# DeepMETv2/DeepMETv2

Hardware: AMD Instinct MI355X
Metric: events/sec (4.5k PF cands, k=16) (higher is better)
Workload: dtype f32

## Files before the change

### deepmetv2_amd/build.py

```python
from __future__ import annotations

import concurrent.futures as cf
import os
import shutil
import subprocess
import sys

PKG_DIR = os.path.dirname(os.path.abspath(__file__))
CSRC = os.path.join(PKG_DIR, "csrc")
OBJ_DIR = os.path.join(CSRC, "_obj")
LIB_PATH = os.path.join(PKG_DIR, "libdmet_hip.so")
SOURCES = ["knn.hip", "radius.hip", "edgeconv.hip", "edgemlp.hip", "misc.hip", "dense.hip", "encoder.hip", "norm.hip", "edgeconv_bwd.hip",
           "head.hip", "finalize.hip", "pool.hip",
           "edgemlp_f32.hip", "edgemlp_bf16.hip", "edgeconv_sum.hip", "gravnet.hip", "attention.hip", "fps.hip", "interpolate.hip",
           "pointnet.hip", "gat.hip", "segment.hip", "multi_aggr.hip", "weighted_sum.hip", "event_norm.hip", "select.hip"]
HEADERS = [os.path.join(CSRC, h) for h in ("common.h", "bn_affine.h", "knn_common.h", "knn_filter.h", "knn_key64.h", "nls_body.h",
                                           "edgemlp_fused.h", "row_softmax.h")] + \
          [os.path.join(PKG_DIR, "..", "include", "dmet.h")]
ARCH = "gfx950"
CXXFLAGS = ["-O3", "-std=c++17", "-fPIC", f"--offload-arch={ARCH}", "-ffp-contract=off", "-Wall",
            "-Wno-unused-function", "-DNDEBUG"]


def _hipcc() -> str:
    exe = shutil.which("hipcc") or "/opt/rocm/bin/hipcc"
    if not os.path.exists(exe):
        raise RuntimeError("hipcc not found: cannot build libdmet_hip.so")
    return exe


def _stale(target: str, deps) -> bool:
    if not os.path.exists(target):
        return True
    t = os.path.getmtime(target)
    return any(os.path.getmtime(d) > t for d in deps if os.path.exists(d))


def _compile(src: str, force: bool) -> str:
    obj = os.path.join(OBJ_DIR, os.path.splitext(src)[0] + ".o")
    path = os.path.join(CSRC, src)
    if force or _stale(obj, [path] + HEADERS):
        cmd = [_hipcc()] + CXXFLAGS + ["-c", path, "-o", obj]
        subprocess.check_call(cmd)
    return obj


def build_hip(force: bool = False, verbose: bool = False) -> str:
    os.makedirs(OBJ_DIR, exist_ok=True)
    with cf.ThreadPoolExecutor(max_workers=min(4, len(SOURCES))) as ex:
        objs = list(ex.map(lambda s: _compile(s, force), SOURCES))
    if force or _stale(LIB_PATH, objs):
        cmd = [_hipcc(), "-shared", "-fPIC", f"--offload-arch={ARCH}", "-o", LIB_PATH] + objs
        if verbose:
            print(" ".join(cmd))
        subprocess.check_call(cmd)
    return LIB_PATH


if __name__ == "__main__":
    print(build_hip(force="--force" in sys.argv, verbose=True))
```

### deepmetv2_amd/csrc/knn.hip

```cpp
#include <stdlib.h>

#include "common.h"
#include "knn_common.h"
#include "knn_key64.h"
#include "nls_body.h"

namespace dmet {
namespace {

constexpr int kTileC = 32;
constexpr int kQMax = 8;
constexpr int kMaxSplit = 8;
constexpr int kWavesPerGroup = 4;

#define DMET_PKSUB_LO " op_sel:[0,0] op_sel_hi:[0,1] neg_lo:[0,1] neg_hi:[0,1]\n\t"
#define DMET_PKSUB_HI " op_sel:[1,0] op_sel_hi:[1,1] neg_lo:[0,1] neg_hi:[0,1]\n\t"
__device__ __forceinline__ void pk_dist_step4(f2 &accA, f2 &accB, f2 vxy, f2 vzw, f2 wxy, f2 wzw, f2 q0, f2 q1, f2 q2,
                                              f2 q3)
{
    f2 t0, t1, t2, t3;
    asm("v_pk_add_f32 %[t0], %[vxy], %[q0]" DMET_PKSUB_LO
        "v_pk_add_f32 %[t1], %[wxy], %[q0]" DMET_PKSUB_LO
        "v_pk_add_f32 %[t2], %[vxy], %[q1]" DMET_PKSUB_HI
        "v_pk_add_f32 %[t3], %[wxy], %[q1]" DMET_PKSUB_HI
        "v_pk_fma_f32 %[a], %[t0], %[t0], %[a]\n\t"
        "v_pk_fma_f32 %[b], %[t1], %[t1], %[b]\n\t"
        "v_pk_add_f32 %[t0], %[vzw], %[q2]" DMET_PKSUB_LO
        "v_pk_add_f32 %[t1], %[wzw], %[q2]" DMET_PKSUB_LO
        "v_pk_fma_f32 %[a], %[t2], %[t2], %[a]\n\t"
        "v_pk_fma_f32 %[b], %[t3], %[t3], %[b]\n\t"
        "v_pk_add_f32 %[t2], %[vzw], %[q3]" DMET_PKSUB_HI
        "v_pk_add_f32 %[t3], %[wzw], %[q3]" DMET_PKSUB_HI
        "v_pk_fma_f32 %[a], %[t0], %[t0], %[a]\n\t"
        "v_pk_fma_f32 %[b], %[t1], %[t1], %[b]\n\t"
        "v_pk_fma_f32 %[a], %[t2], %[t2], %[a]\n\t"
        "v_pk_fma_f32 %[b], %[t3], %[t3], %[b]"
        : [a] "+v"(accA), [b] "+v"(accB), [t0] "=&v"(t0), [t1] "=&v"(t1), [t2] "=&v"(t2), [t3] "=&v"(t3)
        : [vxy] "v"(vxy), [vzw] "v"(vzw), [wxy] "v"(wxy), [wzw] "v"(wzw), [q0] "v"(q0), [q1] "v"(q1), [q2] "v"(q2),
          [q3] "v"(q3));
}

template <bool HI>
__device__ __forceinline__ void pk_sub2(f2 &tA, f2 &tB, f2 v, f2 w, f2 q)
{
    if (HI)
        asm("v_pk_add_f32 %[ta], %[v], %[q]" DMET_PKSUB_HI "v_pk_add_f32 %[tb], %[w], %[q]" DMET_PKSUB_HI
            : [ta] "=&v"(tA), [tb] "=&v"(tB) : [v] "v"(v), [w] "v"(w), [q] "v"(q));
    else
        asm("v_pk_add_f32 %[ta], %[v], %[q]" DMET_PKSUB_LO "v_pk_add_f32 %[tb], %[w], %[q]" DMET_PKSUB_LO
            : [ta] "=&v"(tA), [tb] "=&v"(tB) : [v] "v"(v), [w] "v"(w), [q] "v"(q));
}

__device__ __forceinline__ void pk_fma2(f2 &accA, f2 &accB, f2 tA, f2 tB)
{
    asm("v_pk_fma_f32 %[a], %[ta], %[ta], %[a]\n\t"
        "v_pk_fma_f32 %[b], %[tb], %[tb], %[b]"
        : [a] "+v"(accA), [b] "+v"(accB) : [ta] "v"(tA), [tb] "v"(tB));
}

__device__ __forceinline__ float wrap1(float d, float L)
{
    float a, t;
    asm("v_sub_f32 %[t], %[L], |%[d]|\n\t"
        "v_min_f32 %[a], |%[d]|, %[t]"
        : [a] "=v"(a), [t] "=&v"(t) : [d] "v"(d), [L] "s"(L));
    return a;
}

template <bool HI>
__device__ __forceinline__ void pk_dist_step1_per(f2 &accA, f2 &accB, f2 v, f2 w, f2 q, float L, bool wrap)
{
    f2 tA, tB;
    pk_sub2<HI>(tA, tB, v, w, q);
    if (wrap) {
        tA = f2{wrap1(tA.x, L), wrap1(tA.y, L)};
        tB = f2{wrap1(tB.x, L), wrap1(tB.y, L)};
    }
    pk_fma2(accA, accB, tA, tB);
}

template <int DP, int TQ>
struct KnnShared {
    float4 tile[(kTileC + 1) * DP / 4];
    uint2 queue[TQ][kQMax][kWave];
};

template <int KP>
__device__ __attribute__((noinline)) float drain_queue(const uint2 (*queue)[kWave], int lane, int cnt, bool fresh,
                                                       bool valid, float *__restrict__ ld,
                                                       int32_t *__restrict__ lj)
{
    float d[KP];
    int32_t j[KP];
    if (fresh || !valid) {
#pragma unroll
        for (int p = 0; p < KP; ++p) { d[p] = kKnnSentinel; j[p] = -1; }
    } else {
#pragma unroll
        for (int p = 0; p < KP; p += 4) {
            const float4 v = *reinterpret_cast<const float4 *>(ld + p);
            const int4 w = *reinterpret_cast<const int4 *>(lj + p);
            d[p] = v.x; d[p + 1] = v.y; d[p + 2] = v.z; d[p + 3] = v.w;
            j[p] = w.x; j[p + 1] = w.y; j[p + 2] = w.z; j[p + 3] = w.w;
        }
    }
    int maxcnt = cnt;
#pragma unroll
    for (int off = 32; off > 0; off >>= 1) maxcnt = max(maxcnt, __shfl_xor(maxcnt, off, 64));
    for (int s = 0; s < maxcnt; ++s) {
        if (s < cnt) {
            const uint2 e = queue[s][lane];
            const float nd = __uint_as_float(e.x);
            const int32_t nj = (int32_t)e.y;
            if (nd < d[KP - 1]) {
#pragma unroll
                for (int p = KP - 1; p >= 1; --p) {
                    const bool mq = d[p - 1] > nd;
                    const bool mp = d[p] > nd;
                    const float dn = mq ? d[p - 1] : (mp ? nd : d[p]);
                    const int32_t jn = mq ? j[p - 1] : (mp ? nj : j[p]);
                    d[p] = dn;
                    j[p] = jn;
                }
                if (d[0] > nd) { d[0] = nd; j[0] = nj; }
            }
        }
    }
    if (valid) {
#pragma unroll
        for (int p = 0; p < KP; p += 4) {
            *reinterpret_cast<float4 *>(ld + p) = make_float4(d[p], d[p + 1], d[p + 2], d[p + 3]);
            *reinterpret_cast<int4 *>(lj + p) = make_int4(j[p], j[p + 1], j[p + 2], j[p + 3]);
        }
    }
    return d[KP - 1];
}

#ifdef DMET_KNN_STAMP
__device__ unsigned long long g_knn_stamps[1 << 16][4];
#endif

#ifndef DMET_F2_MIN_NODES
#define DMET_F2_MIN_NODES 800
#endif
constexpr int kF2MinNodes = DMET_F2_MIN_NODES;
constexpr int kFilterMaxSplit = 2;
#ifndef DMET_F2_SPLIT_MIN_NODES
#define DMET_F2_SPLIT_MIN_NODES 2560
#endif
constexpr int kF2SplitMinNodes = DMET_F2_SPLIT_MIN_NODES;
constexpr int kF2MaxNodes = 65536;

struct KnnPlan {
    int total_tiles;
    int n_full;
    int split;
    int form1_events;
};

struct KnnArgs {
    const float *x;
    const int64_t *ptr;
    int B;
    int64_t N;
    int D, k;
    int32_t *nbr;
    float *dist;
    uint16_t *nbr16;
    float *wsd;
    int32_t *wsj;
    const KnnPlan *plan;
    const int32_t *order;
    const int32_t *tile_ptr;
    float *psd;
    int32_t *psj;
    const int32_t *flags;
    int flag_min;
    const int32_t *any;
    const int32_t *qlist;
    const int32_t *pos_of;
    int requery_groups;
    int requery_tile_queries;
};

__device__ __forceinline__ uint16_t local_id16(int32_t j, int ev_lo)
{
    return (uint16_t)(j >= 0 ? (unsigned)(j - ev_lo) : 0xFFFFu);
}

constexpr int kMaxSortedEvents = 4096;

struct KnnPlanOut {
    int tile_queries, simds, max_split;
    int32_t *order, *pos_of, *tile_ptr;
    KnnPlan *plan;
};

__device__ __forceinline__ int xcd_dealt_position(int rank, int B)
{
    if (B < 4 * kNumXcd) return rank;
    const int c = rank % (2 * kNumXcd), g = rank / (2 * kNumXcd);
    const int bin = c < kNumXcd ? c : 2 * kNumXcd - 1 - c;
    const int idx = 2 * g + (c >= kNumXcd ? 1 : 0);
    const int rem = B % (2 * kNumXcd), full = B / (2 * kNumXcd);
    int start = 0;
    for (int b = 0; b < bin; ++b)
        start += 2 * full + (b < min(rem, kNumXcd) ? 1 : 0) + ((rem > kNumXcd && b > 2 * kNumXcd - 1 - rem) ? 1 : 0);
    return start + idx;
}

template <bool XY = false>
__device__ __forceinline__ void knn_plan_body(const int64_t *__restrict__ ptr, int B, const KnnPlanOut &o,
                                              const int64_t *__restrict__ cptr = nullptr)
{
    const int tile_queries = o.tile_queries, simds = o.simds, max_split = o.max_split;
    int32_t *__restrict__ order = o.order, *__restrict__ pos_of = o.pos_of, *__restrict__ tile_ptr = o.tile_ptr;
    KnnPlan *__restrict__ plan = o.plan;
    __shared__ int part[256];
    const int tid = threadIdx.x;
    if (B <= kMaxSortedEvents) {
        for (int b = tid; b < B; b += 256) {
            const int64_t nb = ptr[b + 1] - ptr[b];
            int rank = 0;
            if constexpr (XY) {
                const int64_t xb = nb > 0 ? cptr[b + 1] - cptr[b] : -1;
                for (int c = 0; c < B; ++c) {
                    const int64_t nc = ptr[c + 1] - ptr[c];
                    const int64_t xc = nc > 0 ? cptr[c + 1] - cptr[c] : -1;
                    rank += (xc > xb || (xc == xb && (nc > nb || (nc == nb && c < b)))) ? 1 : 0;
                }
            } else {
                for (int c = 0; c < B; ++c) {
                    const int64_t nc = ptr[c + 1] - ptr[c];
                    rank += (nc > nb || (nc == nb && c < b)) ? 1 : 0;
                }
            }
            const int p = xcd_dealt_position(rank, B);
            order[p] = b;
            pos_of[b] = p;
        }
    } else {
        for (int b = tid; b < B; b += 256) { order[b] = b; pos_of[b] = b; }
    }
    __syncthreads();
    const int chunk = (B + 255) / 256;
    const int lo = min(B, tid * chunk), hi = min(B, lo + chunk);
    int sum = 0, nf1 = 0;
    for (int p = lo; p < hi; ++p) {
        const int b = order[p];
        const int64_t nb = ptr[b + 1] - ptr[b];
        sum += (int)((nb + tile_queries - 1) / tile_queries);
        nf1 += (nb > 0 && !(nb >= kF2MinNodes && nb <= kF2MaxNodes)) ? 1 : 0;
    }
    __shared__ unsigned long long xy_cand;
    __shared__ int xy_events;
    if constexpr (XY) {
        if (tid == 0) { xy_cand = 0ull; xy_events = 0; }
        __syncthreads();
        unsigned long long cand = 0ull;
        int evs = 0;
        for (int p = lo; p < hi; ++p) {
            const int b = order[p];
            if (ptr[b + 1] > ptr[b]) { cand += (unsigned long long)(cptr[b + 1] - cptr[b]); ++evs; }
        }
        if (evs) { atomicAdd(&xy_cand, cand); atomicAdd(&xy_events, evs); }
    }
    __shared__ int wave_tot[4], wave_f1[4];
    const int lane = tid & 63, wv = tid >> 6;
    int incl = sum, f1 = nf1;
#pragma unroll
    for (int off = 1; off < 64; off <<= 1) {
        const int t = __shfl_up(incl, off, 64);
        if (lane >= off) incl += t;
    }
#pragma unroll
    for (int off = 32; off > 0; off >>= 1) f1 += __shfl_xor(f1, off, 64);
    if (lane == 63) wave_tot[wv] = incl;
    if (lane == 0) wave_f1[wv] = f1;
    __syncthreads();
    int base = 0;
    for (int w = 0; w < wv; ++w) base += wave_tot[w];
    part[tid] = base + incl - sum;
    if (tid == 0) {
        const int form1_events = wave_f1[0] + wave_f1[1] + wave_f1[2] + wave_f1[3];
        const int tiles = wave_tot[0] + wave_tot[1] + wave_tot[2] + wave_tot[3];
        int n_full = tiles, split = 1;
        const int full = (tiles / simds) * simds;
        const int rem = tiles - full;
        bool cut = rem > 0;
        if constexpr (XY) cut = cut && xy_events > 0 && xy_cand >= 512ull * (unsigned long long)xy_events;
        else cut = cut && B > 0 && (ptr[B] - ptr[0]) >= (int64_t)512 * B;
        if (cut) {
            int f = simds / rem;
            if (f > max_split) f = max_split;
            if (f >= 2) { n_full = full; split = f; }
        }
        plan->total_tiles = tiles; plan->n_full = n_full; plan->split = split; plan->form1_events = form1_events;
        tile_ptr[B] = tiles;
    }
    __syncthreads();
    int run = part[tid];
    for (int p = lo; p < hi; ++p) {
        const int b = order[p];
        tile_ptr[p] = run;
        run += (int)((ptr[b + 1] - ptr[b] + tile_queries - 1) / tile_queries);
    }
    if (o.max_split == kFilterMaxSplit) {
// ... 968 lines not shown
```

### deepmetv2_amd/csrc/knn_filter.h

```cpp
constexpr int kFQ = 64;

typedef float f32x16 __attribute__((ext_vector_type(16)));
typedef short bf16x8 __attribute__((ext_vector_type(8)));
typedef _Float16 f16x8 __attribute__((ext_vector_type(8)));

struct KnnFilterArgs {
    const float *x;
    const int64_t *ptr;
    int B;
    int64_t N;
    int k;
    float *nrm;
    uint8_t *rec;
    const KnnPlan *plan;
    const int32_t *order;
    const int32_t *pos_of;
    const int32_t *tile_ptr;
    float *psd;
    int32_t *psj;
    int32_t *nbr;
    float *dist;
    uint16_t *nbr16;
    int32_t *flags;
    int32_t *any;
// ... 503 lines not shown
                    df = v.z - qrow[4 * c4 + 2]; dc = __builtin_fmaf(df, df, dc);
                    df = v.w - qrow[4 * c4 + 3]; dc = __builtin_fmaf(df, df, dc);
                }
#pragma unroll
                for (int p = KP - 1; p >= 1; --p) {
                    const bool gq = kd[p - 1] > dc || (kd[p - 1] == dc && kj[p - 1] > j);
                    const bool gp = kd[p] > dc || (kd[p] == dc && kj[p] > j);
                    const float dn = gq ? kd[p - 1] : (gp ? dc : kd[p]);
                    const int32_t jn = gq ? kj[p - 1] : (gp ? j : kj[p]);
                    kd[p] = dn; kj[p] = jn;
                }
                if (kd[0] > dc || (kd[0] == dc && kj[0] > j)) { kd[0] = dc; kj[0] = j; }
            }
        };
        float4 pa[8], pb[8];
        int32_t ja = -1, jb = -1;
        fetch(0, pa, ja);
        fetch(1, pb, jb);
        for (int c = 0; c < maxcnt; c += 2) {
            {
                float4 cur[8];
#pragma unroll
                for (int r = 0; r < 8; ++r) cur[r] = pa[r];
                const int32_t jc = ja;
                if (c + 2 < maxcnt) fetch(c + 2, pa, ja);
                round(cur, jc, c < mycnt);
            }
            if (c + 1 < maxcnt) {
                float4 cur[8];
#pragma unroll
                for (int r = 0; r < 8; ++r) cur[r] = pb[r];
                const int32_t jc = jb;
                if (c + 3 < maxcnt) fetch(c + 3, pb, jb);
                round(cur, jc, c + 1 < mycnt);
            }
        }
        if (valid) {
            const int k = a.k;
            float kth = -1.0f;
#pragma unroll
            for (int p = 0; p < KP; ++p) {
                if (p < k) {
                    a.nbr[(int64_t)myq * k + p] = kj[p];
                    a.dist[(int64_t)myq * k + p] = kd[p];
                }
                if (p == k - 1 && kj[p] >= 0) kth = kd[p];
            }
            if (a.nbr16) {
                uint16_t *r16 = a.nbr16 + (int64_t)myq * k;
                if ((k & 1) == 0) {
#pragma unroll
                    for (int p = 0; p + 1 < KP; p += 2)
                        if (p < k)
                            reinterpret_cast<unsigned *>(r16)[p >> 1] =
                                (unsigned)local_id16(kj[p], ev_lo) | ((unsigned)local_id16(kj[p + 1], ev_lo) << 16);
                } else {
#pragma unroll
                    for (int p = 0; p < KP; ++p)
                        if (p < k) r16[p] = local_id16(kj[p], ev_lo);
                }
            }
            const float tau = L.tk[M - 1];
            const float nx = a.nrm[myq];
            const float an = __builtin_sqrtf(nx) * 1.000001f;
            const float rn = an + __builtin_sqrtf(fmaxf(kth, 0.0f)) * 1.00002f;
            const float slack = 2.0f * (4e-5f * an * rn + 1e-5f * rn * rn + 4e-6f * an * an) + 1e-30f;
            const bool full = tau < kKnnSentinel;
            if (L.overflow || !fits || (full && !(tau + nx - slack > kth))) {
                flag_query(a, myq, a.xtile_ptr[pos] + (myq - ev_lo) / a.xtile_queries);
            }
        }
        return;
    }
    if (a.no_rerank) {
        if (valid && sub == 0) flag_query(a, myq, a.xtile_ptr[pos] + (myq - ev_lo) / a.xtile_queries);
        return;
    }
    if (valid) {
        const int64_t slot = (int64_t)(tile - n_full) * kFQ + hh * 32 + col;
        float *ld = a.psd + (slot * nsub + sub) * MS;
        int32_t *lj = a.psj + (slot * nsub + sub) * MS;
        const float tfin = L.tk[M - 1];
        int out = 0;
        for (int pass = 0; pass < 2; ++pass)
            for (int s = 0; s < L.cnt; ++s) {
                const float key = __uint_as_float(Q.key[s][lane]);
                if ((pass == 0 ? key < tfin : key == tfin) && out < M) {
                    ld[out] = key;
                    lj[out] = ev_lo + (int32_t)Q.id[s][lane];
                    ++out;
                }
            }
        for (; out < M; ++out) { ld[out] = kKnnSentinel; lj[out] = -1; }
        ld[M] = L.tk[M - 1];
        lj[M] = (L.overflow || !fits) ? 1 : 0;
    }
}

template <int KP>
__global__ __launch_bounds__(kWave * kWavesPerGroup, 2) void knn_filter_kernel(const KnnFilterArgs a)
{
    __shared__ FilterQueue<filter_queue_len(filter_list_len(KP))> queue_all[kWavesPerGroup];
    const int wv = __builtin_amdgcn_readfirstlane(threadIdx.x >> 6), lane = threadIdx.x & 63;
    filter1_wave<KP>(a, queue_all[wv], (int)blockIdx.x, wv, lane);
}


#ifndef DMET_F2_DEFER
#define DMET_F2_DEFER 32
#endif
constexpr int kF2Defer = DMET_F2_DEFER;
#ifdef DMET_F2_LEAN
constexpr int kF2Slots = 26;
constexpr int kF2StageRows = 4;
constexpr int kF2WavesPerSimd = 3;
#else
constexpr int kF2Slots = 30;
constexpr int kF2StageRows = kWave;
constexpr int kF2WavesPerSimd = 2;
#endif
constexpr int kF2RowF = 16;
constexpr unsigned kF2TileBits = 11u, kF2TileMask = (1u << kF2TileBits) - 1u;

struct F2Wave {
    uint2 ent[kF2Slots][kWave];
    float rows[kF2StageRows][kF2RowF + 4];
};
#ifndef DMET_F2_LEAN
static_assert(sizeof(F2Wave) == 20480, "two workgroups of four wavefronts fill the CU's 160 KB exactly");
#else
static_assert(sizeof(F2Wave) * 12 <= 163840, "three workgroups of four wavefronts per CU");
#endif

template <int M>
struct F2Lane {
    float tk[M];
    float tau;
    float margin;
    unsigned tq;
    float rep;
    int cnt;
    bool overflow;
};

template <int M>
__device__ __forceinline__ void f2_compact(F2Lane<M> &L, F2Wave &S, int lane, int limit)
{
    const float tauT = __uint_as_float(__float_as_uint(L.tau) & ~kF2TileMask);
    int maxcnt = L.cnt;
#pragma unroll
    for (int off = 32; off > 0; off >>= 1) maxcnt = max(maxcnt, __shfl_xor(maxcnt, off, 64));
    int out = 0;
    for (int s = 0; s < maxcnt; ++s) {
        if (s < L.cnt) {
            const uint2 e = S.ent[s][lane];
            if (!(__uint_as_float(e.y & ~kF2TileMask) > tauT)) { S.ent[out][lane] = e; ++out; }
        }
    }
    L.cnt = out;
    if (out > limit) {
        L.overflow = true;
        L.cnt = 0;
        L.tau = -__builtin_inff();
    }
}

__device__ __forceinline__ f16x8 f2_fold(unsigned tq)
{
    const f16x8 pc = {(_Float16)0.0f, (_Float16)0.0f, (_Float16)0.0f, (_Float16)0.0f, (_Float16)kF2NormP[0],
                      (_Float16)kF2NormP[1], (_Float16)kF2NormP[2], (_Float16)kF2NormP[3]};
    uint4 u = __builtin_bit_cast(uint4, pc);
    u.x = tq;
    return __builtin_bit_cast(f16x8, u);
}

__device__ __forceinline__ void f2_fold_tau(f16x8 (&fq)[2], unsigned tq)
{
    const auto tt = __builtin_amdgcn_permlane32_swap(tq, tq, false, false);
    uint4 u0 = __builtin_bit_cast(uint4, fq[0]), u1 = __builtin_bit_cast(uint4, fq[1]);
    u0.x = tt[0];
    u1.x = tt[1];
    fq[0] = __builtin_bit_cast(f16x8, u0);
    fq[1] = __builtin_bit_cast(f16x8, u1);
}

template <int NH = 1>
struct F2Ops {
    f16x8 a[2 * NH];
    f16x8 f;
};
template <>
struct F2Ops<2> {
    f16x8 a[4];
    f32x16 c;
};

template <int NH = 1>
__device__ __forceinline__ f32x16 f2_block(const F2Ops<NH> &o, const f16x8 (&bv)[2 * NH], const f16x8 &fold)
{
    f32x16 acc;
    if constexpr (NH == 1) acc = __builtin_amdgcn_mfma_f32_32x32x16_f16(o.f, fold, f32x16{}, 0, 0, 0);
    else acc = o.c;
#pragma unroll
    for (int m = 0; m < 2 * NH; ++m) acc = __builtin_amdgcn_mfma_f32_32x32x16_f16(o.a[m], bv[m], acc, 0, 0, 0);
    return acc;
}

template <int NH = 1>
__device__ __forceinline__ void f2_load(F2Ops<NH> &o, const uint8_t *__restrict__ rec, int64_t tidx, int lane, int hh,
                                        unsigned &rofs)
{
    if constexpr (NH == 1) {
        const uint64_t sb = reinterpret_cast<uint64_t>(rec + tidx * rec_bytes(NH));
        const uint64_t ub = ((uint64_t)(unsigned)__builtin_amdgcn_readfirstlane((int)(sb >> 32)) << 32) |
                            (unsigned)__builtin_amdgcn_readfirstlane((int)sb);
        typedef const f16x8 __attribute__((address_space(1))) *GlobalFrag;
        asm volatile("" : "+v"(rofs));
        const GlobalFrag g = (GlobalFrag)(ub + (uint64_t)rofs);
#pragma unroll
        for (int m = 0; m < 2; ++m) o.a[m] = g[m * 64];
        o.f = g[2 * 64];
    } else {
        const uint8_t *base = rec + tidx * rec_bytes(NH);
        const f16x8 *g = reinterpret_cast<const f16x8 *>(base);
#pragma unroll
        for (int m = 0; m < 2 * NH; ++m) o.a[m] = g[m * 64 + lane];
        const float4 *nr = reinterpret_cast<const float4 *>(base + kRec16FragBytes * NH);
#pragma unroll
        for (int q = 0; q < 4; ++q) {
            const float4 v = nr[2 * q + hh];
            o.c[4 * q] = v.x; o.c[4 * q + 1] = v.y; o.c[4 * q + 2] = v.z; o.c[4 * q + 3] = v.w;
        }
    }
}

__device__ __forceinline__ unsigned f2_tau16(float tau, float &rep)
{
    const float x = __builtin_amdgcn_fmed3f(-tau * (1.0f / kF2TauC[0]), -65504.0f, 65504.0f);
    float v = __builtin_amdgcn_fmed3f(__builtin_fmaf(__builtin_fabsf(x), -0x1p-9f, x), -65504.0f, 65504.0f);
    const float y0 = (float)__builtin_amdgcn_cvt_pkrtz(v, v)[0];
    const float w = __builtin_fmaf(-y0, kF2TauC[0] / kF2TauC[1], x * (kF2TauC[0] / kF2TauC[1]));
    v = fminf(__builtin_fmaf(__builtin_fabsf(w), -0x1p-9f, w - 0x1p-24f), 65504.0f);
    const auto y = __builtin_amdgcn_cvt_pkrtz(y0, v);
    rep = -__builtin_fmaf(y0, kF2TauC[0], (float)y[1] * kF2TauC[1]);
    return __builtin_bit_cast(unsigned, y);
}

__device__ __forceinline__ float f2_key_lower(float cmin, float rep)
{
    const float s = cmin + rep;
    return __builtin_fmaf(__builtin_fabsf(s), -0x1p-22f, __builtin_fmaf(__builtin_fabsf(rep), -0x1p-17f, s));
}

template <int NH = 1>
__device__ __forceinline__ float f2_cert_T(float tau)
{
    if constexpr (NH != 1) return tau;
    const float T = fminf(tau, kF2TauRepMax);
    return __builtin_fmaf(__builtin_fabsf(T), -0x1p-16f, T) - 1e-16f;
}
template <int NH = 1>
__device__ __forceinline__ bool f2_full(float tau) { return NH == 1 || tau < kKnnSentinel; }

__device__ __forceinline__ float f2_slack(float an, float rn, float scale)
{
    return 2.0f * scale * (4e-5f * an * rn + 1e-5f * rn * rn + 4e-6f * an * an) + 1.96e-3f * an * rn + 6e-7f * (an + rn) +
           6e-14f * rn * rn + 1e-12f;
}

template <int NH = 1>
__device__ __forceinline__ float f2_cert_threshold(float kth, float nx, float slack)
{
    float ts = kth - nx + slack;
    ts += __builtin_fabsf(ts) * ((NH == 1 ? 0x1p-15f : 0.0f) + 4.8e-7f) + (nx + slack) * 4.8e-7f + (NH == 1 ? 2e-16f : 1e-30f);
    return ts;
}

template <int NH = 1>
__device__ __forceinline__ float f2_cut(float tkk, float nx, float scale)
{
    const float sc = NH == 1 ? 1.0f : 1.5f;
    const float an = __builtin_sqrtf(nx) * 1.000001f;
    const float u0 = fmaxf(tkk + nx, 0.0f);
    float s = f2_slack(an, an + __builtin_sqrtf(u0) * 1.00002f, sc);
    s = f2_slack(an, an + __builtin_sqrtf(u0 + s) * 1.00002f, sc);
    const float U = u0 + s;
    const float ts = f2_cert_threshold<NH>(U, nx, f2_slack(an, an + __builtin_sqrtf(U) * 1.00002f, sc));
    return __builtin_fmaf(scale, ts - tkk, tkk);
}

constexpr int f2_list_len(int KP) { return KP <= 16 ? KP + 6 : KP + 4; }
constexpr int f2_list_cap(int M) { return M <= 22 ? M - 6 : M - 4; }

template <int M>
__device__ __forceinline__ float f2_running_tau(const F2Lane<M> &L)
{
    float t = L.tk[f2_list_cap(M) - 1] + L.margin;
    asm("v_min_f32 %0, %0, %1" : "+v"(t) : "v"(L.tk[M - 1]));
    return t;
}

__device__ __forceinline__ int f2_mask_row(int p) { return (p & 3) + 8 * ((p & 15) >> 2) + 4 * (p >> 4); }

template <int M, bool UPD, bool REC, bool INS, int NH = 1, bool CONV = true, int LEAD = 2>
__device__ __forceinline__ void f2_tile(F2Lane<M> &L, F2Wave &S, const uint8_t *__restrict__ rec, int64_t rbase, int t,
                                        int t_hi, f32x16 &c0, f32x16 &c1, f32x16 &n0, f32x16 &n1, float &rc, float &rn,
                                        const F2Ops<NH> &use, F2Ops<NH> &ld, const f16x8 (&bq)[2][2 * NH], f16x8 (&fq)[2],
                                        int lane, int hh, bool alive, float &carry, unsigned &rofs)
{
#if defined(DMET_F2_ABL) && DMET_F2_ABL >= 2
    constexpr bool kRec = false;
#else
    constexpr bool kRec = REC;
#endif
#if defined(DMET_F2_ABL) && DMET_F2_ABL >= 3
    constexpr bool kUpd = false;
#else
    constexpr bool kUpd = UPD;
#endif
    if (kRec) {
        if (__any(L.cnt >= kF2Slots - 1)) f2_compact<M>(L, S, lane, kF2Slots - 3);
    }
#if defined(DMET_F2_SAMEREC)
    f2_load<NH>(ld, rec, rbase + (t & 1), lane, hh, rofs);
#else
    f2_load<NH>(ld, rec, rbase + min(t + LEAD, t_hi - 1), lane, hh, rofs);
#endif
    n0 = f2_block<NH>(use, bq[0], fq[0]);
    n1 = f2_block<NH>(use, bq[1], fq[1]);
    rn = L.rep;
    unsigned mask = 0u;
    if (kRec) {
        unsigned ma = 0u, mb = 0u;
        if constexpr (NH == 1) {
#pragma unroll
            for (int e = 0; e < 16; ++e) {
                ma = __builtin_amdgcn_alignbit(ma, __float_as_uint(c0[e]), 31);
                mb = __builtin_amdgcn_alignbit(mb, __float_as_uint(c1[e]), 31);
            }
        } else {
            const auto tt = __builtin_amdgcn_permlane32_swap(__float_as_uint(L.tau), __float_as_uint(L.tau), false, false);
            const float t0 = __uint_as_float(tt[0]), t1 = __uint_as_float(tt[1]);
#pragma unroll
            for (int e = 0; e < 16; ++e) {
                ma = __builtin_amdgcn_alignbit(ma, __float_as_uint(c0[e] - t0), 31);
                mb = __builtin_amdgcn_alignbit(mb, __float_as_uint(c1[e] - t1), 31);
            }
        }
        const auto mm = __builtin_amdgcn_permlane32_swap(ma, mb, false, false);
        mask = (mm[0] << 16) | mm[1];
    }
    float tmin = -__builtin_inff();
    if (kUpd) {
        float na, nb;
        asm("v_min3_f32 %0, %1, %2, %3" : "=v"(na) : "s"(kKnnSentinel), "v"(c0[0]), "v"(c0[1]));
        asm("v_min3_f32 %0, %1, %2, %3" : "=v"(nb) : "s"(kKnnSentinel), "v"(c1[0]), "v"(c1[1]));
#pragma unroll
        for (int e = 2; e < 16; e += 2) {
            asm("v_min3_f32 %0, %0, %1, %2" : "+v"(na) : "v"(c0[e]), "v"(c0[e + 1]));
            asm("v_min3_f32 %0, %0, %1, %2" : "+v"(nb) : "v"(c1[e]), "v"(c1[e + 1]));
        }
        const auto nn = __builtin_amdgcn_permlane32_swap(__float_as_uint(na), __float_as_uint(nb), false, false);
        tmin = __uint_as_float(nn[0]);
        asm("v_min_f32 %0, %0, %1" : "+v"(tmin) : "v"(__uint_as_float(nn[1])));
        if (NH == 1 && kRec) tmin = f2_key_lower(tmin, rc);
    }
    if (kRec) {
        const unsigned packed = (__float_as_uint(tmin) & ~kF2TileMask) | (unsigned)t;
        S.ent[L.cnt][lane] = make_uint2(mask, packed);
        L.cnt += (mask != 0u) ? 1 : 0;
    }
    if (kUpd) {
        if (INS) {
            float v = tmin < -3.0e38f ? kKnnSentinel : tmin;
            asm("v_min_f32 %0, %0, %1" : "+v"(v) : "v"(carry));
            carry = kKnnSentinel;
#pragma unroll
            for (int p = M - 1; p >= 1; --p) L.tk[p] = __builtin_amdgcn_fmed3f(L.tk[p - 1], v, L.tk[p]);
            asm("v_min_f32 %0, %0, %1" : "+v"(L.tk[0]) : "v"(v));
            constexpr bool kRun = kRec && (NH != 1 || CONV);
            const float tau = kRun ? f2_running_tau<M>(L) : L.tk[M - 1];
            if (alive && !L.overflow) L.tau = tau;
            if (NH == 1 && kRec && CONV) {
                L.tq = f2_tau16(L.tau, L.rep);
                f2_fold_tau(fq, L.tq);
            }
        } else {
            carry = tmin;
        }
    }
#ifdef DMET_F2_SCHED
#pragma unroll
    for (int g = 0; g < 12; ++g) {
        __builtin_amdgcn_sched_group_barrier(0x008, 1, 0);
        __builtin_amdgcn_sched_group_barrier(0x002, (kRec ? 11 : (kUpd ? 5 : 2)), 0);
    }
#endif
}

template <int M, bool UPD, bool REC, int NH = 1>
__device__ __forceinline__ void f2_sweep(F2Lane<M> &L, F2Wave &S, const uint8_t *__restrict__ rec, int64_t rbase,
                                         int t_lo, int t_hi, const f16x8 (&bq)[2][2 * NH], int lane, int hh, bool alive)
{
    if (t_lo >= t_hi) return;
    F2Ops<NH> A, B;
    unsigned rofs = (unsigned)lane * 16u;
    f2_load<NH>(A, rec, rbase + t_lo, lane, hh, rofs);
    f16x8 fq[2] = {f2_fold(0u), f2_fold(0u)};
    if (NH == 1 && REC) {
        L.tq = f2_tau16(L.tau, L.rep);
        f2_fold_tau(fq, L.tq);
        asm volatile("" : "+v"(fq[0]), "+v"(fq[1]));
    }
    float rc = L.rep, rn;
    f32x16 c0 = f2_block<NH>(A, bq[0], fq[0]);
    f32x16 c1 = f2_block<NH>(A, bq[1], fq[1]);
    f32x16 n0, n1;
    f2_load<NH>(A, rec, rbase + min(t_lo + 1, t_hi - 1), lane, hh, rofs);
    float carry = kKnnSentinel;
    if constexpr (NH == 1 && UPD && REC) {
        F2Ops<NH> C;
        f2_load<NH>(B, rec, rbase + min(t_lo + 2, t_hi - 1), lane, hh, rofs);
        for (int t = t_lo; t < t_hi; t += 6) {
            f2_tile<M, UPD, REC, true, NH, false, 3>(L, S, rec, rbase, t, t_hi, c0, c1, n0, n1, rc, rn, A, C, bq, fq, lane, hh,
                                                     alive, carry, rofs);
            if (t + 1 >= t_hi) break;
            f2_tile<M, UPD, REC, true, NH, true, 3>(L, S, rec, rbase, t + 1, t_hi, n0, n1, c0, c1, rn, rc, B, A, bq, fq, lane,
                                                    hh, alive, carry, rofs);
            if (t + 2 >= t_hi) break;
            f2_tile<M, UPD, REC, true, NH, false, 3>(L, S, rec, rbase, t + 2, t_hi, c0, c1, n0, n1, rc, rn, C, B, bq, fq, lane,
                                                     hh, alive, carry, rofs);
            if (t + 3 >= t_hi) break;
            f2_tile<M, UPD, REC, true, NH, true, 3>(L, S, rec, rbase, t + 3, t_hi, n0, n1, c0, c1, rn, rc, A, C, bq, fq, lane,
                                                    hh, alive, carry, rofs);
            if (t + 4 >= t_hi) break;
            f2_tile<M, UPD, REC, true, NH, false, 3>(L, S, rec, rbase, t + 4, t_hi, c0, c1, n0, n1, rc, rn, B, A, bq, fq, lane,
                                                     hh, alive, carry, rofs);
            if (t + 5 >= t_hi) break;
            f2_tile<M, UPD, REC, true, NH, true, 3>(L, S, rec, rbase, t + 5, t_hi, n0, n1, c0, c1, rn, rc, C, B, bq, fq, lane,
                                                    hh, alive, carry, rofs);
        }
        return;
    }
    for (int t = t_lo; t < t_hi; t += 2) {
        f2_tile<M, UPD, REC, true, NH, false>(L, S, rec, rbase, t, t_hi, c0, c1, n0, n1, rc, rn, A, B, bq, fq, lane, hh, alive,
                                              carry, rofs);
        if (t + 1 < t_hi)
            f2_tile<M, UPD, REC, true, NH, true>(L, S, rec, rbase, t + 1, t_hi, n0, n1, c0, c1, rn, rc, B, A, bq, fq, lane, hh,
                                                 alive, carry, rofs);
    }
}

__device__ __forceinline__ int filter_group(const KnnFilterArgs &a)
{
    const int full_groups = a.plan->n_full / kWavesPerGroup;
    return (int)blockIdx.x < full_groups ? xcd_swizzle((int)blockIdx.x, full_groups) : (int)blockIdx.x;
}

template <int KP, int NH = 1>
__device__ __forceinline__ void filter2_wave(const KnnFilterArgs &a, F2Wave &S, int *tickets, int group, int wv, int lane)
{
    constexpr int M = f2_list_len(KP);
    static_assert(f2_list_cap(M) == KP, "f2_running_tau reads slot KP - 1 of the list");
    constexpr int D = 32 * NH;
    constexpr int MS = (M + 1 + 3) & ~3;
    const int col = lane & 31, hh = lane >> 5;
    const uint8_t *__restrict__ rec = a.rec;
    const int64_t *__restrict__ ptr = a.ptr;

    const int n_full = a.plan->n_full, split = a.plan->split, total = a.plan->total_tiles;
    const int item = group * kWavesPerGroup + wv;
    int tile = item, sub = 0, nsub = 1;
    if (item >= n_full) {
        const int r = item - n_full;
        tile = n_full + r / split;
        sub = r % split;
        nsub = split;
    }
    if (tile >= total) return;
    const int pos = find_tile_event(a.tile_ptr, a.B, tile);
    const int ev = a.order[pos];
    const int ev_lo = (int)ptr[ev], ev_hi = (int)ptr[ev + 1];
    const int q_first = ev_lo + (tile - a.tile_ptr[pos]) * kFQ;
    if (!f2_in_domain(ev_hi - ev_lo)) {
        if (NH != 1 && sub == 0) {
            const int q = q_first + lane;
            if (q < ev_hi) {
                flag_query(a, q, a.xtile_ptr[pos] + (q - ev_lo) / a.xtile_queries);
            }
        }
        return;
    }
    int clo = ev_lo, chi = ev_hi;
    if (nsub > 1) {
        if (ev_hi - ev_lo < kF2SplitMinNodes) {
            if (sub != 0) return;
            nsub = 1;
        } else {
            const int chunk = (((chi - clo) + nsub - 1) / nsub + 31) & ~31;
            clo = min(chi, clo + sub * chunk);
            chi = min(chi, clo + chunk);
        }
    }
    const int64_t rbase = (ptr[ev] >> 5) + ev;
    const int64_t rlast = rbase + (ev_hi - ev_lo - 1) / 32;
    const int t_lo = (clo - ev_lo) / 32, t_hi = (chi - ev_lo + 31) / 32;

    const int myq = q_first + hh * 32 + col;
    const bool valid = myq < ev_hi;
    float t_fix = -__builtin_inff();
    bool act = valid;
    for (int attempt = 0;; ++attempt) {
    F2Lane<M> L;
#pragma unroll
    for (int p = 0; p < M; ++p) L.tk[p] = kKnnSentinel;
    L.tau = attempt == 0 ? -__builtin_inff() : t_fix;
    L.margin = __builtin_inff();
    L.tq = 0u;
    L.rep = 0.0f;
    L.cnt = 0;
    L.overflow = false;
    {
        f16x8 bq[2][2 * NH];
#pragma unroll
        for (int b = 0; b < 2; ++b) {
            const int64_t qrec = min(rbase + (q_first - ev_lo) / 32 + b, rlast);
            const f16x8 *g = reinterpret_cast<const f16x8 *>(rec + qrec * rec_bytes(NH));
#pragma unroll
            for (int m = 0; m < 2 * NH; ++m) bq[b][m] = g[m * 64 + lane] * (_Float16)-2.0f;
        }
        if (attempt == 0) {
            const int t_def = min(t_hi, t_lo + kF2Defer);
            f2_sweep<M, true, false, NH>(L, S, rec, rbase, t_lo, t_def, bq, lane, hh, valid);
            if (a.run_cut && a.cut_scale >= 0.0f && a.k == KP && t_def < t_hi) {
                const float tkk = L.tk[KP - 1];
                int qi = valid ? myq : ev_lo;
                asm volatile("" : "+v"(qi));
                const float m = f2_cut<NH>(tkk, a.nrm[qi], a.cut_scale) - tkk;
                if (tkk < kKnnSentinel && m > 0.0f && m < __builtin_inff()) L.margin = __builtin_fmaf(m, 0.01f, m);
                L.tau = fminf(L.tau, tkk + L.margin);
            }
            f2_sweep<M, true, true, NH>(L, S, rec, rbase, t_def, t_hi, bq, lane, hh, valid);
            if (a.cut_scale >= 0.0f) {
                float tkk = kKnnSentinel;
#pragma unroll
                for (int p = 0; p < KP; ++p)
                    if (p == a.k - 1) tkk = L.tk[p];
                if (tkk < kKnnSentinel) {
                    int qi = valid ? myq : ev_lo;
                    asm volatile("" : "+v"(qi));
                    const float cut = f2_cut<NH>(tkk, a.nrm[qi], a.cut_scale);
                    L.tau = fminf(L.tau, cut);
                }
            }
            f2_sweep<M, false, true, NH>(L, S, rec, rbase, t_lo, t_def, bq, lane, hh, valid);
        } else {
            f2_sweep<M, false, true, NH>(L, S, rec, rbase, t_lo, t_hi, bq, lane, hh, valid);
        }
    }
    f2_compact<M>(L, S, lane, kF2Slots);
#if defined(DMET_F2_ABL) && DMET_F2_ABL >= 1
    return;
#endif

    const int64_t qrow_id = valid ? myq : ev_lo;
    float qrow[D];
    {
        const float4 *g = reinterpret_cast<const float4 *>(a.x + qrow_id * D);
#pragma unroll
        for (int c = 0; c < D / 4; ++c) {
            const float4 v = g[c];
            qrow[4 * c] = v.x; qrow[4 * c + 1] = v.y; qrow[4 * c + 2] = v.z; qrow[4 * c + 3] = v.w;
        }
    }
    static_assert(__builtin_bit_cast(unsigned, kKnnSentinel) == kKey64SentinelBits, "knn_key64.h clamps to the sentinel");
    double kk[KP];
#pragma unroll
    for (int p = 0; p < KP; ++p) kk[p] = key64_as_double(kKey64Empty);
    const int nent = (act && !L.overflow) ? L.cnt : 0;
    int slot = 0;
    unsigned cmask = 0u;
    int ctile = 0;
    uint2 enext = S.ent[0][lane];
    auto pop = [&]() __attribute__((always_inline)) -> int32_t {
        const bool take = cmask == 0u && slot < nent;
        cmask = take ? enext.x : cmask;
        ctile = take ? (int)(enext.y & kF2TileMask) : ctile;
        slot += take ? 1 : 0;
        enext = S.ent[min(slot, kF2Slots - 1)][lane];
        int32_t jl = -1;
        if (cmask != 0u) {
            const int r = __builtin_clz(cmask);
            cmask &= ~(0x80000000u >> r);
            jl = ctile * 32 + f2_mask_row(r);
        }
        return jl;
    };
    const float4 *x4 = reinterpret_cast<const float4 *>(a.x);
#ifdef DMET_RR_PRIO
    __builtin_amdgcn_s_setprio(DMET_RR_PRIO);
#endif
    if constexpr (NH != 1) {
        for (;;) {
            const int32_t jl = pop();
            if (!__any(jl >= 0)) break;
            const int32_t j = ev_lo + jl;
            const float4 *row = x4 + (int64_t)(jl >= 0 ? j : ev_lo) * (D / 4);
            float4 v[D / 4];
#pragma unroll
            for (int c = 0; c < D / 4; ++c) v[c] = row[c];
            float dc = 0.0f;
#pragma unroll
            for (int c = 0; c < D / 4; ++c) {
                float df;
                df = v[c].x - qrow[4 * c + 0]; dc = __builtin_fmaf(df, df, dc);
                df = v[c].y - qrow[4 * c + 1]; dc = __builtin_fmaf(df, df, dc);
                df = v[c].z - qrow[4 * c + 2]; dc = __builtin_fmaf(df, df, dc);
                df = v[c].w - qrow[4 * c + 3]; dc = __builtin_fmaf(df, df, dc);
            }
            key64_insert<KP>(kk, key64_word(__float_as_uint(dc), (unsigned)j, jl >= 0));
        }
    } else {
    struct HalfRows { float4 v0, v1, v2, v3, v4, v5, v6, v7; };
#ifdef DMET_RR_FULLROW
    auto fetch = [&](int32_t jl) __attribute__((always_inline)) -> HalfRows {
        const int32_t jc = ev_lo + (jl >= 0 ? jl : 0);
        const int64_t o = lane & 7;
        const int sub = lane >> 3;
        HalfRows R;
        R.v0 = x4[(int64_t)__shfl(jc, 0 + sub, 64) * 8 + o];
        R.v1 = x4[(int64_t)__shfl(jc, 8 + sub, 64) * 8 + o];
        R.v2 = x4[(int64_t)__shfl(jc, 16 + sub, 64) * 8 + o];
        R.v3 = x4[(int64_t)__shfl(jc, 24 + sub, 64) * 8 + o];
        R.v4 = x4[(int64_t)__shfl(jc, 32 + sub, 64) * 8 + o];
        R.v5 = x4[(int64_t)__shfl(jc, 40 + sub, 64) * 8 + o];
        R.v6 = x4[(int64_t)__shfl(jc, 48 + sub, 64) * 8 + o];
        R.v7 = x4[(int64_t)__shfl(jc, 56 + sub, 64) * 8 + o];
        return R;
    };
#else
    const uint64_t xb = reinterpret_cast<uint64_t>(a.x + (int64_t)ev_lo * D);
    const uint64_t xbs = ((uint64_t)(unsigned)__builtin_amdgcn_readfirstlane((int)(xb >> 32)) << 32) |
                         (unsigned)__builtin_amdgcn_readfirstlane((int)xb);
    typedef float f32x4 __attribute__((ext_vector_type(4)));
    typedef const f32x4 __attribute__((address_space(1))) *GlobalRow;
    auto ld = [](GlobalRow g, int i) __attribute__((always_inline)) -> float4 {
        const f32x4 v = g[i];
        return make_float4(v.x, v.y, v.z, v.w);
    };
    auto fetch = [&](int32_t jl) __attribute__((always_inline)) -> HalfRows {
        const int32_t jc = jl >= 0 ? jl : 0;
        const unsigned o = 16u * (lane & 3);
        const GlobalRow r0 = (GlobalRow)(xbs + (uint64_t)(((unsigned)__shfl(jc, 0 + (lane >> 2), 64) << 7) + o));
        const GlobalRow r1 = (GlobalRow)(xbs + (uint64_t)(((unsigned)__shfl(jc, 16 + (lane >> 2), 64) << 7) + o));
        const GlobalRow r2 = (GlobalRow)(xbs + (uint64_t)(((unsigned)__shfl(jc, 32 + (lane >> 2), 64) << 7) + o));
        const GlobalRow r3 = (GlobalRow)(xbs + (uint64_t)(((unsigned)__shfl(jc, 48 + (lane >> 2), 64) << 7) + o));
        HalfRows R;
        R.v0 = ld(r0, 0); R.v1 = ld(r1, 0); R.v2 = ld(r2, 0); R.v3 = ld(r3, 0);
        R.v4 = ld(r0, 4); R.v5 = ld(r1, 4); R.v6 = ld(r2, 4); R.v7 = ld(r3, 4);
        return R;
    };
#endif
    auto chain16 = [&](float dc, int h) __attribute__((always_inline)) -> float {
#pragma unroll
        for (int c4 = 0; c4 < 4; ++c4) {
            const float4 v = *reinterpret_cast<const float4 *>(&S.rows[lane][4 * c4]);
            const int f0 = 16 * h + 4 * c4;
            float df;
            df = v.x - qrow[f0 + 0]; dc = __builtin_fmaf(df, df, dc);
            df = v.y - qrow[f0 + 1]; dc = __builtin_fmaf(df, df, dc);
            df = v.z - qrow[f0 + 2]; dc = __builtin_fmaf(df, df, dc);
            df = v.w - qrow[f0 + 3]; dc = __builtin_fmaf(df, df, dc);
        }
        return dc;
    };
    auto round = [&](const HalfRows &R, int32_t jl) __attribute__((always_inline)) {
#ifdef DMET_RR_FULLROW
        float4 *dst = reinterpret_cast<float4 *>(&S.rows[lane >> 3][4 * (lane & 3)]);
        constexpr int kS8 = 8 * (kF2RowF + 4) / 4;
        const bool lowhalf = (lane & 4) == 0;
        wave_sync();
        if (lowhalf) {
            dst[0] = R.v0; dst[kS8] = R.v1; dst[2 * kS8] = R.v2; dst[3 * kS8] = R.v3;
            dst[4 * kS8] = R.v4; dst[5 * kS8] = R.v5; dst[6 * kS8] = R.v6; dst[7 * kS8] = R.v7;
        }
        wave_sync();
        float dc = chain16(0.0f, 0);
        wave_sync();
        if (!lowhalf) {
            dst[0] = R.v0; dst[kS8] = R.v1; dst[2 * kS8] = R.v2; dst[3 * kS8] = R.v3;
            dst[4 * kS8] = R.v4; dst[5 * kS8] = R.v5; dst[6 * kS8] = R.v6; dst[7 * kS8] = R.v7;
        }
        wave_sync();
        dc = chain16(dc, 1);
#else
        float4 *dst = reinterpret_cast<float4 *>(&S.rows[lane >> 2][4 * (lane & 3)]);
        constexpr int kStride = 16 * (kF2RowF + 4) / 4;
        wave_sync();
        dst[0] = R.v0; dst[kStride] = R.v1; dst[2 * kStride] = R.v2; dst[3 * kStride] = R.v3;
        wave_sync();
        float dc = chain16(0.0f, 0);
        wave_sync();
        dst[0] = R.v4; dst[kStride] = R.v5; dst[2 * kStride] = R.v6; dst[3 * kStride] = R.v7;
        wave_sync();
        dc = chain16(dc, 1);
#endif
        key64_insert<KP>(kk, key64_word(__float_as_uint(dc), (unsigned)(ev_lo + jl), jl >= 0));
    };
#ifdef DMET_RR_THREE
    constexpr bool kThreeRounds = KP <= 16;
#else
    constexpr bool kThreeRounds = false;
#endif
    if constexpr (kThreeRounds) {
        int32_t ja = pop(), jb, jc;
        HalfRows pa = fetch(ja), pb, pc;
        jb = pop();
        pb = fetch(jb);
        for (;;) {
            if (!__any(ja >= 0)) break;
            jc = pop(); pc = fetch(jc);
            round(pa, ja);
            if (!__any(jb >= 0)) break;
            ja = pop(); pa = fetch(ja);
            round(pb, jb);
            if (!__any(jc >= 0)) break;
            jb = pop(); pb = fetch(jb);
            round(pc, jc);
        }
    } else {
        int32_t ja = pop(), jb;
        HalfRows pa = fetch(ja), pb;
        for (;;) {
            if (!__any(ja >= 0)) break;
            jb = pop(); pb = fetch(jb);
            round(pa, ja);
            if (!__any(jb >= 0)) break;
            ja = pop(); pa = fetch(ja);
            round(pb, jb);
        }
    }
    }
#ifdef DMET_RR_PRIO
    __builtin_amdgcn_s_setprio(0);
#endif
    float kd[KP];
    int32_t kj[KP];
#pragma unroll
    for (int p = 0; p < KP; ++p) {
        kd[p] = __uint_as_float((unsigned)(key64_as_word(kk[p]) >> 32));
        kj[p] = kd[p] == kKnnSentinel ? -1 : (int32_t)(unsigned)key64_as_word(kk[p]);
    }
// ... 341 lines not shown
```

Before: 51450.

## Deepen KNN filter record prefetch to four rotating operand sets

Replaces the three-buffer, lead-3 rotation in the recording filter sweep with a four-set ring of operand buffers whose load lead equals the set count. It now also covers the non-update recording path. This hides more global-load latency behind the MFMA distance blocks. The cost is more live VGPRs, which may reduce occupancy or cause spills. The load-tile schedule is factored into a small shared header.

```diff
diff --git a/deepmetv2_amd/build.py b/deepmetv2_amd/build.py
--- a/deepmetv2_amd/build.py
+++ b/deepmetv2_amd/build.py
@@ -14,7 +14,8 @@
            "head.hip", "finalize.hip", "pool.hip",
            "edgemlp_f32.hip", "edgemlp_bf16.hip", "edgeconv_sum.hip", "gravnet.hip", "attention.hip", "fps.hip", "interpolate.hip",
            "pointnet.hip", "gat.hip", "segment.hip", "multi_aggr.hip", "weighted_sum.hip", "event_norm.hip", "select.hip"]
-HEADERS = [os.path.join(CSRC, h) for h in ("common.h", "bn_affine.h", "knn_common.h", "knn_filter.h", "knn_key64.h", "nls_body.h",
+HEADERS = [os.path.join(CSRC, h) for h in ("common.h", "bn_affine.h", "knn_common.h", "knn_filter.h", "knn_key64.h", "knn_tile_schedule.h",
+                                           "nls_body.h",
                                            "edgemlp_fused.h", "row_softmax.h")] + \
           [os.path.join(PKG_DIR, "..", "include", "dmet.h")]
 ARCH = "gfx950"
diff --git a/deepmetv2_amd/csrc/knn.hip b/deepmetv2_amd/csrc/knn.hip
--- a/deepmetv2_amd/csrc/knn.hip
+++ b/deepmetv2_amd/csrc/knn.hip
@@ -3,6 +3,7 @@
 #include "common.h"
 #include "knn_common.h"
 #include "knn_key64.h"
+#include "knn_tile_schedule.h"
 #include "nls_body.h"
 
 namespace dmet {
diff --git a/deepmetv2_amd/csrc/knn_filter.h b/deepmetv2_amd/csrc/knn_filter.h
--- a/deepmetv2_amd/csrc/knn_filter.h
+++ b/deepmetv2_amd/csrc/knn_filter.h
@@ -829,9 +829,9 @@
 
 __device__ __forceinline__ int f2_mask_row(int p) { return (p & 3) + 8 * ((p & 15) >> 2) + 4 * (p >> 4); }
 
-template <int M, bool UPD, bool REC, bool INS, int NH = 1, bool CONV = true, int LEAD = 2>
+template <int M, bool UPD, bool REC, bool INS, int NH = 1, bool CONV = true>
 __device__ __forceinline__ void f2_tile(F2Lane<M> &L, F2Wave &S, const uint8_t *__restrict__ rec, int64_t rbase, int t,
-                                        int t_hi, f32x16 &c0, f32x16 &c1, f32x16 &n0, f32x16 &n1, float &rc, float &rn,
+                                        int t_load, f32x16 &c0, f32x16 &c1, f32x16 &n0, f32x16 &n1, float &rc, float &rn,
                                         const F2Ops<NH> &use, F2Ops<NH> &ld, const f16x8 (&bq)[2][2 * NH], f16x8 (&fq)[2],
                                         int lane, int hh, bool alive, float &carry, unsigned &rofs)
 {
@@ -851,7 +851,7 @@
 #if defined(DMET_F2_SAMEREC)
     f2_load<NH>(ld, rec, rbase + (t & 1), lane, hh, rofs);
 #else
-    f2_load<NH>(ld, rec, rbase + min(t + LEAD, t_hi - 1), lane, hh, rofs);
+    f2_load<NH>(ld, rec, rbase + t_load, lane, hh, rofs);
 #endif
     n0 = f2_block<NH>(use, bq[0], fq[0]);
     n1 = f2_block<NH>(use, bq[1], fq[1]);
@@ -925,56 +925,67 @@
 #endif
 }
 
+template <int M, bool UPD>
+__device__ __forceinline__ void f2_sweep4(F2Lane<M> &L, F2Wave &S, const uint8_t *__restrict__ rec, int64_t rbase, int t_lo,
+                                          int t_hi, const f16x8 (&bq)[2][2], int lane, int hh, bool alive)
+{
+    F2Ops<1> s[kF2Sets];
+    unsigned rofs = (unsigned)lane * 16u;
+#pragma unroll
+    for (int j = 0; j < kF2Sets; ++j) f2_load<1>(s[f2_tile_set(j)], rec, rbase + f2_load_tile(t_lo, j, t_hi), lane, hh, rofs);
+    f16x8 fq[2] = {f2_fold(0u), f2_fold(0u)};
+    L.tq = f2_tau16(L.tau, L.rep);
+    f2_fold_tau(fq, L.tq);
+    asm volatile("" : "+v"(fq[0]), "+v"(fq[1]));
+    float rc = L.rep, rn;
+    f32x16 c0 = f2_block<1>(s[0], bq[0], fq[0]);
+    f32x16 c1 = f2_block<1>(s[0], bq[1], fq[1]);
+    f32x16 n0, n1;
+    float carry = kKnnSentinel;
+    static_assert(f2_tile_set(4) == 0 && f2_tile_key_block(2) == 0 && f2_tile_key_block(3) == 1 && !f2_call_converts(2) &&
+                      f2_call_converts(3),
+                  "the trip below is the schedule's, written out");
+    for (int t = t_lo;;) {
+        f2_tile<M, UPD, true, true, 1, false>(L, S, rec, rbase, t, f2_load_tile(t, kF2Sets, t_hi), c0, c1, n0, n1, rc, rn, s[1],
+                                              s[0], bq, fq, lane, hh, alive, carry, rofs);
+        if (++t >= t_hi) break;
+        f2_tile<M, UPD, true, true, 1, true>(L, S, rec, rbase, t, f2_load_tile(t, kF2Sets, t_hi), n0, n1, c0, c1, rn, rc, s[2],
+                                             s[1], bq, fq, lane, hh, alive, carry, rofs);
+        if (++t >= t_hi) break;
+        f2_tile<M, UPD, true, true, 1, false>(L, S, rec, rbase, t, f2_load_tile(t, kF2Sets, t_hi), c0, c1, n0, n1, rc, rn, s[3],
+                                              s[2], bq, fq, lane, hh, alive, carry, rofs);
+        if (++t >= t_hi) break;
+        f2_tile<M, UPD, true, true, 1, true>(L, S, rec, rbase, t, f2_load_tile(t, kF2Sets, t_hi), n0, n1, c0, c1, rn, rc, s[0],
+                                             s[3], bq, fq, lane, hh, alive, carry, rofs);
+        if (++t >= t_hi) break;
+    }
+}
+
 template <int M, bool UPD, bool REC, int NH = 1>
 __device__ __forceinline__ void f2_sweep(F2Lane<M> &L, F2Wave &S, const uint8_t *__restrict__ rec, int64_t rbase,
                                          int t_lo, int t_hi, const f16x8 (&bq)[2][2 * NH], int lane, int hh, bool alive)
 {
     if (t_lo >= t_hi) return;
+    if constexpr (NH == 1 && REC) {
+        f2_sweep4<M, UPD>(L, S, rec, rbase, t_lo, t_hi, bq, lane, hh, alive);
+        return;
+    }
     F2Ops<NH> A, B;
     unsigned rofs = (unsigned)lane * 16u;
     f2_load<NH>(A, rec, rbase + t_lo, lane, hh, rofs);
     f16x8 fq[2] = {f2_fold(0u), f2_fold(0u)};
-    if (NH == 1 && REC) {
-        L.tq = f2_tau16(L.tau, L.rep);
-        f2_fold_tau(fq, L.tq);
-        asm volatile("" : "+v"(fq[0]), "+v"(fq[1]));
-    }
     float rc = L.rep, rn;
     f32x16 c0 = f2_block<NH>(A, bq[0], fq[0]);
     f32x16 c1 = f2_block<NH>(A, bq[1], fq[1]);
     f32x16 n0, n1;
-    f2_load<NH>(A, rec, rbase + min(t_lo + 1, t_hi - 1), lane, hh, rofs);
+    f2_load<NH>(A, rec, rbase + f2_load_tile(t_lo, 1, t_hi), lane, hh, rofs);
     float carry = kKnnSentinel;
-    if constexpr (NH == 1 && UPD && REC) {
-        F2Ops<NH> C;
-        f2_load<NH>(B, rec, rbase + min(t_lo + 2, t_hi - 1), lane, hh, rofs);
-        for (int t = t_lo; t < t_hi; t += 6) {
-            f2_tile<M, UPD, REC, true, NH, false, 3>(L, S, rec, rbase, t, t_hi, c0, c1, n0, n1, rc, rn, A, C, bq, fq, lane, hh,
-                                                     alive, carry, rofs);
-            if (t + 1 >= t_hi) break;
-            f2_tile<M, UPD, REC, true, NH, true, 3>(L, S, rec, rbase, t + 1, t_hi, n0, n1, c0, c1, rn, rc, B, A, bq, fq, lane,
-                                                    hh, alive, carry, rofs);
-            if (t + 2 >= t_hi) break;
-            f2_tile<M, UPD, REC, true, NH, false, 3>(L, S, rec, rbase, t + 2, t_hi, c0, c1, n0, n1, rc, rn, C, B, bq, fq, lane,
-                                                     hh, alive, carry, rofs);
-            if (t + 3 >= t_hi) break;
-            f2_tile<M, UPD, REC, true, NH, true, 3>(L, S, rec, rbase, t + 3, t_hi, n0, n1, c0, c1, rn, rc, A, C, bq, fq, lane,
-                                                    hh, alive, carry, rofs);
-            if (t + 4 >= t_hi) break;
-            f2_tile<M, UPD, REC, true, NH, false, 3>(L, S, rec, rbase, t + 4, t_hi, c0, c1, n0, n1, rc, rn, B, A, bq, fq, lane,
-                                                     hh, alive, carry, rofs);
-            if (t + 5 >= t_hi) break;
-            f2_tile<M, UPD, REC, true, NH, true, 3>(L, S, rec, rbase, t + 5, t_hi, n0, n1, c0, c1, rn, rc, C, B, bq, fq, lane,
-                                                    hh, alive, carry, rofs);
-        }
-        return;
-    }
     for (int t = t_lo; t < t_hi; t += 2) {
-        f2_tile<M, UPD, REC, true, NH, false>(L, S, rec, rbase, t, t_hi, c0, c1, n0, n1, rc, rn, A, B, bq, fq, lane, hh, alive,
-                                              carry, rofs);
+        f2_tile<M, UPD, REC, true, NH, false>(L, S, rec, rbase, t, f2_load_tile(t, kF2PlainLead, t_hi), c0, c1, n0, n1, rc, rn,
+                                              A, B, bq, fq, lane, hh, alive, carry, rofs);
         if (t + 1 < t_hi)
-            f2_tile<M, UPD, REC, true, NH, true>(L, S, rec, rbase, t + 1, t_hi, n0, n1, c0, c1, rn, rc, B, A, bq, fq, lane, hh,
-                                                 alive, carry, rofs);
+            f2_tile<M, UPD, REC, true, NH, true>(L, S, rec, rbase, t + 1, f2_load_tile(t + 1, kF2PlainLead, t_hi), n0, n1, c0,
+                                                 c1, rn, rc, B, A, bq, fq, lane, hh, alive, carry, rofs);
     }
 }
 
diff --git a/deepmetv2_amd/csrc/knn_tile_schedule.h b/deepmetv2_amd/csrc/knn_tile_schedule.h
--- /dev/null
+++ b/deepmetv2_amd/csrc/knn_tile_schedule.h
@@ -0,0 +1,16 @@
+#pragma once
+
+#if defined(__HIPCC__) || defined(__CUDACC__)
+#define DMET_SCHED_FN __host__ __device__ inline
+#else
+#define DMET_SCHED_FN inline
+#endif
+
+constexpr int kF2Sets = 4;
+constexpr int kF2PlainLead = 2;
+
+DMET_SCHED_FN constexpr int f2_load_tile(int t, int lead, int t_hi) { return t + lead < t_hi - 1 ? t + lead : t_hi - 1; }
+
+DMET_SCHED_FN constexpr int f2_tile_set(int i) { return i & (kF2Sets - 1); }
+DMET_SCHED_FN constexpr int f2_tile_key_block(int i) { return i & 1; }
+DMET_SCHED_FN constexpr bool f2_call_converts(int i) { return (i & 1) != 0; }
```

New measurement: 52450, median of 6. 1.9% higher.
